# loli/medpy

Measured on AMD Instinct MI355X. Metric: Mvoxels/s graph-cut (build+solve), 512^3 6-conn; fraction of HBM roofline, higher is better.
Workload: dtype f64

## Files before the change

medpy_amd/csrc/mgc_common.h:

```cpp
#ifndef MGC_COMMON_H
#define MGC_COMMON_H

#include <stdint.h>

#if defined(__HIPCC__)
#define MGC_HD __host__ __device__ __forceinline__
#else
#define MGC_HD inline
#endif

#define MGC_T 8
#define MGC_TV 512
#define MGC_TF 64
#define MGC_HINF 0x3f3f3f3f

#define MGC_NDIR 6
#define MGC_MASK_SINK 0x40
#define MGC_NCOUNT 32
#define MGC_ST_SETTLED 1u
#define MGC_ST_SINK 2u
#define MGC_ST_DIRTY 4u
#define MGC_ST_SUSPECT 8u
#define MGC_ST_EXCESS 16u
#define MGC_ST_ALLINF 32u
#define MGC_ST_SOURCE 64u
#define MGC_WALL_WEIGHT 9.313225746154785e-10
#define MGC_WALL_VOXELS 24
#define MGC_ST_DEP_SHIFT 8
#define MGC_CNT_SINK_TILES 13
#define MGC_CNT_WALL_TILES 12
#define MGC_CNT_RADIAL_C 14
#define MGC_CNT_SOURCE_OPEN 15
#define MGC26_CNT_RADIAL_C 26
#define MGC26_CNT_SOURCE_OPEN 27
#define MGC_CNT_CHANGED 21
#define MGC_CNT_FILTER 22
#define MGC_CNT_FILTER_ACT 23
#define MGC_CNT_FILTER_B 30
#define MGC_CNT_FILTER_ACT_B 31
#define MGC_CNT_DEFERRED 28
#define MGC_CNT_WAVE_TILES 29
#define MGC_CNT_NOT_FULL 28

#if defined(__HIP_DEVICE_COMPILE__)
#define MGC_STORE_STREAM(p, v) __builtin_nontemporal_store((v), (p))
#else
#define MGC_STORE_STREAM(p, v) (*(p) = (v))
#endif

struct MgcLattice {
    int64_t dz, dy, dx;
    int64_t nvox;
    int gz, gy, gx;
    int ntiles;
    int tz_own_lo, tz_own_hi;
    int tz_global0;
    double*   rcap;
    double*   cap0;
    double*   excess;
    double*   sink;
    int32_t*  height;
    uint8_t*  rmask;
    uint32_t* rmask32;
    int       ndir;
    double*   obox;
    uint32_t* oflags;
    int32_t*  list[20];
    int32_t*  count;
    int32_t*  scount;
    int       nshard;
    int       shard_cap;
    uint32_t* stamp;
    uint32_t* rstamp;
    uint32_t* status;
    int       halo_max_rec;
    int32_t*  hshadow[2];
    unsigned long long* prof;
    const uint8_t* tsrc;
};

#ifndef MGC_NSHARD
#define MGC_NSHARD 1
#endif

MGC_HD int mgc_cnt_radial_c(const MgcLattice& L) { return L.ndir == 26 ? MGC26_CNT_RADIAL_C : MGC_CNT_RADIAL_C; }
MGC_HD int mgc_cnt_source_open(const MgcLattice& L) { return L.ndir == 26 ? MGC26_CNT_SOURCE_OPEN : MGC_CNT_SOURCE_OPEN; }

MGC_HD int32_t* mgc_counter(const MgcLattice& L, int c, int shard) { return L.scount + c * L.nshard + shard; }
// ... 112 lines not shown
```

medpy_amd/csrc/mgc_kernels.hip:

```cpp
#include <hip/hip_runtime.h>
#include <rccl/rccl.h>

#include <dlfcn.h>

#include <math.h>
#include <stdarg.h>
#include <stdio.h>
#include <stdlib.h>
#include <string.h>

#include <algorithm>
#include <chrono>
#include <map>
#include <string>
#include <mutex>
#include <thread>
#include <vector>

#include "../../include/medpy_hip.h"
#include "mgc_tile_ops.inl"
#include "mgc_tile_ops26.inl"
#include "mgc_wave_ops.inl"
#include "mgc_wave_ops26.inl"
#include "mgc_dt_ops.inl"
// ... 620 lines not shown
        __syncthreads();
    }
    x.flush_marks(L);
}

__global__ __launch_bounds__(MGC_TV) void k_absorb(MgcLattice L)
{
    __shared__ MgcTileShared S;
    GpuBlock x(S);
    for (int tile = blockIdx.x; tile < L.ntiles; tile += gridDim.x) {
        x.new_tile();
        mgc_absorb_tile(x, L, tile);
        __syncthreads();
    }
}

__global__ __launch_bounds__(MGC_TV) void k_relabel_all(MgcLattice L, uint32_t epoch, int next_list)
{
    __shared__ MgcTileShared S;
    GpuBlock x(S);
    int visited = 0;
    for (int tile = blockIdx.x; tile < L.ntiles; tile += gridDim.x) {
        x.new_tile();
        visited += (L.status[tile] >> 1) & 1u;
        mgc_relabel_tile(x, L, tile, epoch, next_list, true);
        __syncthreads();
    }
    if (threadIdx.x == 0 && visited) atomicAdd(&L.count[9], visited);
}

__global__ __launch_bounds__(MGC_TV) void k_relabel_list(MgcLattice L, int lst, uint32_t epoch, int next_list, int zero_list)
{
    __shared__ MgcTileShared S;
    GpuBlock x(S);
    MgcListView view;
    const int n = mgc_list_view(L, lst, view);
    if (blockIdx.x == 0 && threadIdx.x == 0 && n) atomicAdd(&L.count[9], n);
    mgc_clear_counter(L, zero_list);
    for (int i = blockIdx.x; i < n; i += gridDim.x) {
        x.new_tile();
        mgc_relabel_tile(x, L, mgc_list_at(L, lst, view, i), epoch, next_list, false);
        __syncthreads();
    }
}

__global__ void k_zero_counts(MgcLattice L, uint32_t mask)
{
    const int c = (int)threadIdx.x / MGC_NSHARD, sh = (int)threadIdx.x % MGC_NSHARD;
    if (!((mask >> c) & 1u)) return;
    if (sh == 0) L.count[c] = 0;
    if (sh < L.nshard) *mgc_counter(L, c, sh) = 0;
}

__global__ void k_status_or(MgcLattice L, uint32_t bits, uint32_t clear)
{
    const int tile = blockIdx.x * blockDim.x + threadIdx.x;
    if (tile < L.ntiles) L.status[tile] = (L.status[tile] & ~clear) | bits;
}

template <bool FULL>
__global__ __launch_bounds__(MGC_TV) void k_suspect_pass(MgcLattice L)
{
    const int bxn = (L.gx + 7) / 8, byn = (L.gy + 7) / 8, bzn = (L.gz + 7) / 8;
    const int t = threadIdx.x;
    bool any = false;
    for (int b = blockIdx.x; b < bxn * byn * bzn; b += gridDim.x) {
        const int bx = b % bxn, by = (b / bxn) % byn, bz = b / (bxn * byn);
        const int tz = bz * 8 + (t >> 6), ty = by * 8 + ((t >> 3) & 7), tx = bx * 8 + (t & 7);
        const bool in = tz < L.gz && ty < L.gy && tx < L.gx;
        const int tile = in ? mgc_tile_id(L, tz, ty, tx) : 0;
        for (int it = 0; it < 24; ++it) {
            const bool ch = in && (FULL ? mgc26_suspect_tile(L, tile) : mgc_suspect_tile(L, tile));
            any |= ch;
            __threadfence_block();
            if (!__syncthreads_or(ch)) break;
        }
    }
    if (any) L.count[MGC_CNT_CHANGED] = 1;
}

template <bool FULL>
__global__ __launch_bounds__(MGC_TV) void k_reset_suspect(MgcLattice L, uint32_t epoch, int list, int bricks)
{
    __shared__ MgcTileShared S;
    __shared__ int sel[MGC_TV];
    __shared__ int nsel;
    GpuBlock x(S);
    for (int base = blockIdx.x * MGC_TV; base < L.ntiles; base += gridDim.x * MGC_TV) {
        if (threadIdx.x == 0) nsel = 0;
        __syncthreads();
        const int mine = base + (int)threadIdx.x;
        if (mine < L.ntiles && (L.status[mine] & MGC_ST_SUSPECT)) sel[atomicAdd(&nsel, 1)] = mine;
        __syncthreads();
        const int n = nsel;
        for (int i = 0; i < n; ++i) {
            L.height[(int64_t)sel[i] * MGC_TV + threadIdx.x] = MGC_HINF;
            if (threadIdx.x < MGC_TF) mgc_shadow_reset(L, sel[i], (int)threadIdx.x);
        }
        if ((int)threadIdx.x < n) {
            const int tile = sel[threadIdx.x];
            L.status[tile] = (L.status[tile] & ~(MGC_ST_SUSPECT | MGC_ST_DIRTY | MGC_ST_SETTLED | (FULL ? MGC26_ST_DEP_MASK : (63u << MGC_ST_DEP_SHIFT)))) | MGC_ST_ALLINF;
            if (bricks) mgc_enqueue_brick(x, L, list, epoch, mgc_brick_of_tile(L, tile));
            else mgc_enqueue(x, L, list, L.rstamp, epoch, tile);
        }
        __syncthreads();
    }
}

__global__ void k_filter(MgcLattice L, int mode, int list, int cnt)
{
    for (int base = blockIdx.x * blockDim.x; base < L.ntiles; base += gridDim.x * blockDim.x) {
        const int tile = base + (int)threadIdx.x;
        bool take = false;
        if (tile < L.ntiles && mgc_owned(L, tile)) {
            if (mode == 0) {
                int tz, ty, tx;
                mgc_tile_coords(L, tile, tz, ty, tx);
                for (int f = 0; f < 6 && !take; ++f) {
                    const int nt = mgc_tile_nbr(L, tz, ty, tx, f);
                    take = nt >= 0 && ((L.oflags[nt] >> (f ^ 1)) & 1u);
                }
            } else if (mode == 1) {
                take = (L.status[tile] & (MGC_ST_EXCESS | MGC_ST_ALLINF)) == MGC_ST_EXCESS;
            } else if (mode == 3) {
                take = (L.status[tile] & MGC_ST_SINK) != 0;
            } else {
                take = (L.status[tile] & MGC_ST_SUSPECT) != 0;
            }
        }
        const unsigned long long m = __ballot(take);
        if (m) {
            int pos = 0;
            const int sh = (int)(blockIdx.x & (unsigned)(L.nshard - 1));
            if ((threadIdx.x & 63) == 0) pos = atomicAdd(mgc_counter(L, cnt, sh), __popcll(m));
            pos = __shfl(pos, 0);
            if (take) L.list[list][(int64_t)sh * L.shard_cap + pos + __popcll(m & ((1ull << (threadIdx.x & 63)) - 1ull))] = tile;
        }
    }
}

__global__ __launch_bounds__(MGC_TV) void k_relabel_first_list(MgcLattice L, int list, int cnt, uint32_t epoch, int next_list)
{
    __shared__ MgcTileShared S;
    GpuBlock x(S);
    MgcListView view;
    const int n = mgc_list_view(L, cnt, view);
    if (blockIdx.x == 0 && threadIdx.x == 0 && n) atomicAdd(&L.count[9], n);
    for (int i = blockIdx.x; i < n; i += gridDim.x) {
        x.new_tile();
        mgc_relabel_tile(x, L, mgc_list_at(L, list, view, i), epoch, next_list, true);
        __syncthreads();
    }
}

__global__ __launch_bounds__(256) void k_absorb_w(MgcLattice L, int list, int cnt, int clear_cnt)
{
    __shared__ MgcWaveShared S;
    GpuWave w(S);
// ... 1528 lines not shown
            *(void**)(&pop) = dlsym(dl, "roctxRangePop");
            if (push && pop) return;
            push = nullptr; pop = nullptr;
        }
    }
};
static MgcRoctx g_roctx;
static inline void mgc_range_push(const char* name)
{
    if (!g_roctx.tried) g_roctx.resolve();
    if (g_roctx.push) (void)g_roctx.push(name);
}
static inline void mgc_range_pop()
{
    if (g_roctx.pop) (void)g_roctx.pop();
}
struct MgcRange {
    explicit MgcRange(const char* name) { mgc_range_push(name); }
    ~MgcRange() { mgc_range_pop(); }
};
static std::string g_create_error;

struct mgc_graph {
    int device = 0;
    int ndim = 0;
    int64_t shape[3] = {1, 1, 1};
    int64_t nvox = 0;
    hipStream_t stream = nullptr;
    hipEvent_t ev[4] = {nullptr, nullptr, nullptr, nullptr};
    std::vector<hipEvent_t> ev_pool;
    struct OpSpan { int a, b, kind; };
    std::vector<hipEvent_t> op_ev;
    std::vector<OpSpan> op_spans;
    MgcLattice L{};
    void* d_image = nullptr; int img_dtype = 0; int term = MGC_TERM_NONE; double sigma = 0; double spacing[3] = {1, 1, 1};
    int has_spacing = 0;
    void* d_prob = nullptr; int prob_dtype = 0; double alpha = 0;
    void* d_lut = nullptr; int lut_n = 0;
    uint8_t* d_fg = nullptr; uint8_t* d_bg = nullptr;
    double* d_tr_in = nullptr; double flow_const_in = 0;
    MgcBuildArgs build_args{};
    int64_t n_edges = 0, n_runs = 0; int64_t* d_eslot = nullptr; double* d_eval = nullptr; int64_t* d_erun = nullptr;
    bool range_set = false; double range[3] = {0, 0, 0};
    bool edges_applied = false;
    double* d_dense = nullptr;
    std::vector<double*> dense_extra[26];
    int dense_given[26] = {};
    const double** d_dense_planes = nullptr;
    std::map<const void*, size_t> buf_cap;
    uint8_t* d_tsum = nullptr;
    uint8_t* d_tflags = nullptr;
    double* d_tr0 = nullptr; double* d_part = nullptr; double* d_part2 = nullptr; double* d_scalar = nullptr; uint8_t* d_labels = nullptr;
    int32_t* h_count = nullptr;
    double* h_scalar = nullptr;
    uint8_t* h_labels = nullptr; bool labels_on_host = false;
    uint8_t* d_labels_prev = nullptr; bool has_prev = false;
    bool built = false, solved = false;
    bool unconverged = false;
    bool labels_valid = false;
    void* d_vout = nullptr;
    uint16_t* d_dt16 = nullptr;
    uint16_t* d_ds16 = nullptr;
    int32_t* d_hexact = nullptr;
    bool radial_on = false;
    int radial_cycle_no = 0;
    bool all_residual = false;
    int exact_sink_tiles = 1;
    int sink_tiles = 0;
    int wall_tiles = 0;
    int radial_min_walls = 16;
    int sink_sweeps = 8;
    int use_bricks = 0;
    bool brick_mode = false;
    int use_dt = 1;
    int rank = 0, nranks = 1;
    int64_t plane0 = 0, plane1 = 0, own0 = 0, own1 = 0;
    int64_t gd0 = 0;
    uint16_t* d_carry[2] = {nullptr, nullptr};
    uint16_t* d_carry_in[2] = {nullptr, nullptr};
    uint16_t* dt_cur = nullptr;
    void* d_halo = nullptr; int64_t halo_cap = 0;
    ncclComm_t comm = nullptr; void* d_xchg[4] = {nullptr, nullptr, nullptr, nullptr}; int64_t xchg_cap = 0;
    int64_t* d_cnt64 = nullptr;
    double flow_const = 0.0, flow = 0.0;
    MgcSolveParams params = mgc_default_params();
    int grid_cap = 4096;
    int grid26_dis = 16384;
    int wave_kernels = 9;
    int wave_grid_dis = 0, wave_grid_rel = 0;
    int tk_dis = MGC_CNT_TICKET_DIS, tk_rel = MGC_CNT_TICKET_REL;
    int est_phase_tiles = 1 << 30;
    int sweeps_sparse26 = 5;
    int wave_grid26 = 0;
    bool rounds_set = false, sparse26_set = false, wave_set = false;
    bool w26_auto = false;
    int prepush = 1;
    int w26_passes = 2, w26_raises = 1, w26_flags = 0;
    int activate_exact_max = 4096;
    int wave_stagger = 0;
    int64_t launches[MGC_NLAUNCH] = {};
    int repeat_steps = 1;
    int repeat_min_tiles = 0;
    int repeat_flood_min_tiles = 200000;
    bool repeat_now = false;
    int wave_min_tiles = 512;
    uint32_t zero_mask = 0;
// ... 103 lines not shown
    }
    return hipFree(p);
}

template <class T>
static int mgc_alloc(mgc_handle h, T** p, int64_t count)
{
    MGC_HIP(h, mgc_dmalloc((void**)p, (size_t)count * sizeof(T)));
    h->device_bytes += count * (int64_t)sizeof(T);
    return MGC_OK;
}

static void mgc_fold_counts(mgc_handle h)
{
    const int ns = h->L.nshard;
    for (int c = 0; c < MGC_NCOUNT; ++c)
        for (int sh = 0; sh < ns; ++sh) h->h_count[c] += h->h_count[MGC_NCOUNT + c * ns + sh];
}

template <bool FULL>
struct HipDevT {
    mgc_handle h;
    hipError_t first_error = hipSuccess;
    float discharge_ms = 0.f, relabel_ms = 0.f, once_ms = 0.f;
    int64_t discharge_launches = 0, relabel_launches = 0, readbacks = 0;
    int last_discharged = -1;
    int suspect_batch() const { return 4; }
    bool labels_inexact() const { return false; }
    void range_push(const char* name) { mgc_range_push(name); }
    void range_pop() { mgc_range_pop(); }
    struct Span { int a, b, kind; };
    std::vector<Span> spans;
    void check(hipError_t e) { if (e != hipSuccess && first_error == hipSuccess) first_error = e; }
    int grid(int64_t n) const { return (int)(n < 1 ? 1 : (n < h->grid_cap ? n : h->grid_cap)); }
    void fill_heights_inf()
    {
        flush_zero();
        h->labels_valid = true;
        check(hipMemsetAsync(h->L.height, 0x3f, (size_t)h->L.ntiles * MGC_TV * sizeof(int32_t), h->stream));
        hipLaunchKernelGGL(k_status_or, dim3((h->L.ntiles + 255) / 256), dim3(256), 0, h->stream, h->L, (uint32_t)MGC_ST_ALLINF, (uint32_t)MGC_ST_SETTLED);
        for (int sd = 0; sd < 2; ++sd)
            if (h->L.hshadow[sd]) check(hipMemsetAsync(h->L.hshadow[sd], 0x3f, (size_t)h->L.gy * h->L.gx * MGC_TF * sizeof(int32_t), h->stream));
    }
    void flush_zero()
    {
        if (h->pending_zero >= 0) h->zero_mask |= 1u << h->pending_zero;
        h->pending_zero = -1;
        if (h->zero_mask) {
            hipLaunchKernelGGL(k_zero_counts, dim3(1), dim3(MGC_NCOUNT * MGC_NSHARD), 0, h->stream, h->L, h->zero_mask);
            check(hipGetLastError());
        }
        h->zero_mask = 0;
    }
    void zero_count(int i)
    {
        if (i == last_discharged) { flush_zero(); h->pending_zero = i; last_discharged = -1; return; }
        if (h->pending_zero >= 0) { h->zero_mask |= 1u << h->pending_zero; h->pending_zero = -1; }
        h->zero_mask |= 1u << i;
    }
    void read_counts(int* out)
    {
        flush_zero();
        check(hipMemcpyAsync(h->h_count, h->L.count, MGC_NCOUNT * (1 + MGC_NSHARD) * sizeof(int32_t), hipMemcpyDeviceToHost, h->stream));
        check(hipStreamSynchronize(h->stream));
        mgc_fold_counts(h);
        memcpy(out, h->h_count, MGC_NCOUNT * sizeof(int32_t));
        readbacks++;
        if (!FULL) {
            int m = out[6] / 2;
            for (int i = 0; i < 4; ++i) m = out[i] > m ? out[i] : m;
            h->est_phase_tiles = m;
        } else {
            int m = out[MGC26_CNT_ACTIVE] / 8;
            for (int i = 0; i < MGC26_NLIST; ++i) m = out[i] > m ? out[i] : m;
            h->est_phase_tiles = m;
        }
    }
    int filter_grid() const { const int g = (h->L.ntiles + 255) / 256; return g < 1024 ? g : 1024; }
    int fslot(int which) const { return which == 0 ? (h->filt[0] ? MGC_CNT_FILTER_B : MGC_CNT_FILTER) : (h->filt[1] ? MGC_CNT_FILTER_ACT_B : MGC_CNT_FILTER_ACT); }
    int fnext(int which) const { return which == 0 ? (h->filt[0] ? MGC_CNT_FILTER : MGC_CNT_FILTER_B) : (h->filt[1] ? MGC_CNT_FILTER_ACT : MGC_CNT_FILTER_ACT_B); }
    void filter_done(int which, bool consumer_cleared_next)
    {
        if (!consumer_cleared_next) zero_count(fnext(which));
        h->filt[which] ^= 1;
    }
    void absorb_all()
    {
        flush_zero();
        if constexpr (FULL) return;
        else if (!(h->use_filters & 1)) { hipLaunchKernelGGL(k_absorb, dim3(grid(h->L.ntiles)), dim3(MGC_TV), 0, h->stream, h->L); check(hipGetLastError()); }
        else {
            flush_zero();
            hipLaunchKernelGGL(k_filter, dim3(filter_grid()), dim3(256), 0, h->stream, h->L, 0, 6, fslot(0));
            if (h->wave_kernels & 1) hipLaunchKernelGGL(k_absorb_w, dim3(grid((h->L.ntiles + 3) / 4)), dim3(256), 0, h->stream, h->L, 6, fslot(0), fnext(0));
            else hipLaunchKernelGGL(k_absorb_list, dim3(grid(h->L.ntiles)), dim3(MGC_TV), 0, h->stream, h->L, 6, fslot(0), fnext(0));
            filter_done(0, true);
            check(hipGetLastError());
        }
    }
    void relabel_all(uint32_t epoch, int next)
    {
        flush_zero();
        h->brick_mode = false;
        const int id = time_begin(1);
        if constexpr (FULL) hipLaunchKernelGGL(k26_relabel_all, dim3(grid(h->L.ntiles)), dim3(MGC_TV), 0, h->stream, h->L, epoch, next);
        else if (!(h->use_filters & 1)) { hipLaunchKernelGGL(k_relabel_all, dim3(grid(h->L.ntiles)), dim3(MGC_TV), 0, h->stream, h->L, epoch, next); h->launches[MGC_LAUNCH_RELABEL_TILE]++; }
        else {
            flush_zero();
            hipLaunchKernelGGL(k_filter, dim3(filter_grid()), dim3(256), 0, h->stream, h->L, 3, 6, fslot(0));
            if (h->wave_kernels & 8) { hipLaunchKernelGGL(k_relabel_v, dim3(grid(h->L.ntiles)), dim3(MGC_TV / MGC_RELABEL_V), 0, h->stream, h->L, 6, fslot(0), epoch, next, fnext(0), 1); filter_done(0, true); h->launches[MGC_LAUNCH_RELABEL_V]++; }
            else if (h->wave_kernels & 2) { hipLaunchKernelGGL(k_relabel_w, dim3(h->wave_grid_rel), dim3(MGCW_LANES), 0, h->stream, h->L, 6, fslot(0), epoch, next, -1, 1, h->tk_rel); h->tk_rel ^= 1; filter_done(0, false); h->launches[MGC_LAUNCH_RELABEL_W]++; }
            else { hipLaunchKernelGGL(k_relabel_first_list, dim3(grid(h->L.ntiles)), dim3(MGC_TV), 0, h->stream, h->L, 6, fslot(0), epoch, next); filter_done(0, false); h->launches[MGC_LAUNCH_RELABEL_TILE]++; }
        }
        check(hipGetLastError());
        time_end(id);
        relabel_launches++;
    }
    template <int AXIS, int SEED, int FINAL>
    void dt_axis(const void* in, uint16_t* T, int c_min)
// ... 61 lines not shown
        check(hipMemsetAsync(L.count + mgc_cnt_radial_c(L), 0x3f, sizeof(int32_t), h->stream));
        hipLaunchKernelGGL(k_dt_cmin, g(L.ntiles), blk, 0, h->stream, L);
        dt_axis<0, 2, 0>((const void*)L.excess, T, 0);
        dt_axis<1, 0, 0>((const void*)T, T, 0);
        dt_axis<2, 0, 2>((const void*)T, T, c_min);
        std::swap(h->L.height, h->d_hexact);
        check(hipGetLastError());
        time_end(id);
        relabel_launches++;
        return true;
    }
    void radial_save_exact()
    {
        flush_zero();
        check(hipMemcpyAsync(h->d_hexact, h->L.height, (size_t)h->L.ntiles * MGC_TV * sizeof(int32_t), hipMemcpyDeviceToDevice, h->stream));
    }
    void radial_restore_exact()
    {
        flush_zero();
        std::swap(h->L.height, h->d_hexact);
    }
    void radial_lower(int c_min)
    {
        flush_zero();
        const int id = time_begin(2);
        hipLaunchKernelGGL(k_dt_lower, dim3(grid((h->L.ntiles + 3) / 4)), dim3(256), 0, h->stream, h->L, (const uint16_t*)h->d_ds16, c_min);
        check(hipGetLastError());
        time_end(id);
        relabel_launches++;
    }
    void source_open()
    {
        flush_zero();
        hipLaunchKernelGGL(k_source_open, dim3(grid((h->L.ntiles + 3) / 4)), dim3(256), 0, h->stream, h->L);
        check(hipGetLastError());
    }
    void relabel_list(int lst, uint32_t epoch, int next, int zero_list = -1)
    {
        flush_zero();
        const int id = time_begin(1);
        if (!FULL && h->brick_mode) { hipLaunchKernelGGL(k_relabel_b, dim3(grid(mgc_brick_count(h->L))), dim3(MGC_TV), 0, h->stream, h->L, lst, epoch, next, zero_list); h->launches[MGC_LAUNCH_RELABEL_TILE]++; }
        else if constexpr (FULL) hipLaunchKernelGGL(k26_relabel_list, dim3(grid(h->L.ntiles)), dim3(MGC_TV), 0, h->stream, h->L, lst, epoch, next);
        else if (h->wave_kernels & 8) { hipLaunchKernelGGL(k_relabel_v, dim3(grid(h->L.ntiles)), dim3(MGC_TV / MGC_RELABEL_V), 0, h->stream, h->L, lst, lst, epoch, next, zero_list, 0); h->launches[MGC_LAUNCH_RELABEL_V]++; }
        else if (h->wave_kernels & 2) { hipLaunchKernelGGL(k_relabel_w, dim3(h->wave_grid_rel), dim3(MGCW_LANES), 0, h->stream, h->L, lst, lst, epoch, next, zero_list, 0, h->tk_rel); h->tk_rel ^= 1; h->launches[MGC_LAUNCH_RELABEL_W]++; }
        else { hipLaunchKernelGGL(k_relabel_list, dim3(grid(h->L.ntiles)), dim3(MGC_TV), 0, h->stream, h->L, lst, epoch, next, zero_list); h->launches[MGC_LAUNCH_RELABEL_TILE]++; }
        check(hipGetLastError());
        time_end(id);
        relabel_launches++;
    }
    void suspect_pass()
    {
        flush_zero();
        const int nb = ((h->L.gx + 7) / 8) * ((h->L.gy + 7) / 8) * ((h->L.gz + 7) / 8);
        hipLaunchKernelGGL(k_suspect_pass<FULL>, dim3(nb < 4096 ? nb : 4096), dim3(MGC_TV), 0, h->stream, h->L);
        check(hipGetLastError());
    }
    void reset_suspect(uint32_t epoch, int list)
    {
        flush_zero();
        const int id = time_begin(1);
        h->brick_mode = !FULL && h->use_bricks && h->nranks == 1 && !(h->use_filters & 4);
        if (FULL || !(h->use_filters & 4)) hipLaunchKernelGGL(k_reset_suspect<FULL>, dim3(grid((h->L.ntiles + MGC_TV - 1) / MGC_TV)), dim3(MGC_TV), 0, h->stream, h->L, epoch, list, h->brick_mode ? 1 : 0);
        else {
            flush_zero();
            hipLaunchKernelGGL(k_filter, dim3(filter_grid()), dim3(256), 0, h->stream, h->L, 2, 6, fslot(0));
            hipLaunchKernelGGL(k_reset_suspect_list, dim3(grid(h->L.ntiles)), dim3(MGC_TV), 0, h->stream, h->L, 6, fslot(0), epoch, list);
            filter_done(0, false);
        }
        check(hipGetLastError());
        time_end(id);
        relabel_launches++;
    }
    void activate_all(uint32_t phase)
    {
        flush_zero();
        if constexpr (FULL) {
            if (h->L.nshard == 1 && (h->use_filters & 2)) hipLaunchKernelGGL(k26_activate_w, dim3(grid((h->L.ntiles + 3) / 4)), dim3(256), 0, h->stream, h->L, phase);
            else hipLaunchKernelGGL(k26_activate, dim3(grid(h->L.ntiles)), dim3(MGC_TV), 0, h->stream, h->L, phase);
        }
        else if (!(h->use_filters & 2)) hipLaunchKernelGGL(k_activate, dim3(grid(h->L.ntiles)), dim3(MGC_TV), 0, h->stream, h->L, phase);
        else {
            flush_zero();
            hipLaunchKernelGGL(k_filter, dim3(filter_grid()), dim3(256), 0, h->stream, h->L, 1, 7, fslot(1));
            if (h->wave_kernels & 1) { hipLaunchKernelGGL(k_activate_w, dim3(grid((h->L.ntiles + 3) / 4)), dim3(256), 0, h->stream, h->L, 7, fslot(1), phase, h->activate_exact_max, fnext(1)); filter_done(1, true); }
            else { hipLaunchKernelGGL(k_activate_list, dim3(grid(h->L.ntiles)), dim3(MGC_TV), 0, h->stream, h->L, 7, fslot(1), phase); filter_done(1, false); }
        }
        check(hipGetLastError());
    }
    void discharge(int lst, uint32_t phase, int cycles, int sweeps)
    {
        const int zero_idx = h->pending_zero;
        h->pending_zero = -1;
        flush_zero();
        const bool wave_form = !FULL && (h->wave_kernels & 1) && h->est_phase_tiles >= h->wave_min_tiles;
        const int id = time_begin(FULL || wave_form ? 0 : 3);
        if constexpr (FULL) {
            if (h->sweeps_sparse26 > 0 && (int64_t)h->est_phase_tiles * 40 < h->L.ntiles) sweeps = h->sweeps_sparse26;
            if (((h->wave_kernels & 32) || h->w26_auto) && cycles < 0) {
                hipLaunchKernelGGL(k26_discharge_w, dim3(h->wave_grid26), dim3(MGCW_LANES), 0, h->stream, h->L, lst, phase, sweeps, h->w26_auto ? 1 : h->w26_passes, h->w26_raises, h->w26_flags, h->tk_dis, zero_idx);
                h->tk_dis ^= 1;
                h->launches[MGC_LAUNCH_DISCHARGE26_W]++;
            }
            else if (h->wave_kernels & 16) { hipLaunchKernelGGL(k26_discharge_v, dim3(grid(h->L.ntiles)), dim3(MGC_TV / 2), 0, h->stream, h->L, lst, phase, cycles, sweeps, zero_idx); h->launches[MGC_LAUNCH_DISCHARGE26_V]++; }
            else { hipLaunchKernelGGL(k26_discharge, dim3(h->grid26_dis > 0 ? (h->grid26_dis < h->L.ntiles ? h->grid26_dis : h->L.ntiles) : grid(h->L.ntiles)), dim3(MGC_TV), 0, h->stream, h->L, lst, phase, cycles, sweeps, zero_idx); h->launches[MGC_LAUNCH_DISCHARGE26]++; }
        }
        else if (wave_form) {
            const bool exact_sink = h->exact_sink_tiles == 2 || (h->exact_sink_tiles == 1 && 2 * (int64_t)h->sink_tiles > h->L.ntiles);
// ... 396 lines not shown
        L.tz_own_lo = slab->own_lo; L.tz_own_hi = slab->own_hi; L.tz_global0 = slab->tz_global0;
        h->rank = slab->rank; h->nranks = slab->nranks;
        h->plane0 = slab->plane0; h->plane1 = slab->plane1; h->own0 = slab->own0; h->own1 = slab->own1;
    } else {
        h->plane0 = h->own0 = 0; h->plane1 = h->own1 = L.dz;
    }
    h->gd0 = gd0 > 0 ? gd0 : L.dz;
    *out = h;
    MGC_HIP(h, hipSetDevice(device));
    MGC_HIP(h, hipStreamCreateWithFlags(&h->stream, hipStreamNonBlocking));
    for (int i = 0; i < 4; ++i) MGC_HIP(h, hipEventCreate(&h->ev[i]));
    const int64_t nt = L.ntiles, nv = nt * MGC_TV;
    int rc;
    if ((rc = mgc_alloc(h, &L.rcap, nv * L.ndir))) return rc;
    L.cap0 = nullptr;
    if ((rc = mgc_alloc(h, &L.excess, nv))) return rc;
    if ((rc = mgc_alloc(h, &L.sink, nv))) return rc;
    if ((rc = mgc_alloc(h, &L.height, nv))) return rc;
    if (L.ndir == 6) {
        if ((rc = mgc_alloc(h, &L.rmask, nv))) return rc;
        if ((rc = mgc_alloc(h, &L.obox, nt * 6 * MGC_TF))) return rc;
    } else {
        if ((rc = mgc_alloc(h, &L.rmask32, nv))) return rc;
    }
    if ((rc = mgc_alloc(h, &L.oflags, nt))) return rc;
    if (slab && L.ndir == 6) {
        for (int sd = 0; sd < 2; ++sd) {
            if ((rc = mgc_alloc(h, &L.hshadow[sd], (int64_t)L.gy * L.gx * MGC_TF))) return rc;
            MGC_HIP(h, hipMemsetAsync(L.hshadow[sd], 0x3f, (size_t)L.gy * L.gx * MGC_TF * sizeof(int32_t), h->stream));
        }
    }
    L.nshard = 1;
    {
        const int64_t T = gy * gx;
        L.halo_max_rec = (int)(T / 8 > 64 ? T / 8 : (T < 64 ? T : 64));
    }
    L.shard_cap = (int)nt;
    for (int i = 0; i < (L.ndir == 6 ? 8 : 18); ++i)
        if ((rc = mgc_alloc(h, &L.list[i], nt * MGC_NSHARD))) return rc;
    if ((rc = mgc_alloc(h, &L.count, (int64_t)MGC_NCOUNT * (1 + MGC_NSHARD)))) return rc;
    L.scount = L.count + MGC_NCOUNT;
    if ((rc = mgc_alloc(h, &L.stamp, nt))) return rc;
    if ((rc = mgc_alloc(h, &L.rstamp, nt))) return rc;
    if ((rc = mgc_alloc(h, &L.status, nt))) return rc;
    if ((rc = mgc_alloc(h, &h->d_tr0, nv))) return rc;
    if ((rc = mgc_alloc(h, &h->d_tflags, nt))) return rc;
    if ((rc = mgc_alloc(h, &h->d_tsum, nt))) return rc;
    if ((rc = mgc_alloc(h, &h->d_part, nt > 4096 ? nt : (int64_t)4096))) return rc;
    if ((rc = mgc_alloc(h, &h->d_part2, (int64_t)256))) return rc;
    if ((rc = mgc_alloc(h, &h->d_scalar, (int64_t)8))) return rc;
    if ((rc = mgc_alloc(h, &h->d_labels, n))) return rc;
    MGC_HIP(h, hipHostMalloc((void**)&h->h_count, MGC_NCOUNT * (1 + MGC_NSHARD) * sizeof(int32_t), hipHostMallocDefault));
    MGC_HIP(h, hipHostMalloc((void**)&h->h_scalar, 8 * sizeof(double), hipHostMallocDefault));
    MGC_HIP(h, hipMemsetAsync(L.count, 0, MGC_NCOUNT * (1 + MGC_NSHARD) * sizeof(int32_t), h->stream));
    MGC_HIP(h, hipStreamSynchronize(h->stream));
    if (const char* wv = getenv("MEDPY_HIP_WAVE")) { h->wave_kernels = atoi(wv); h->wave_set = true; }
    {
        hipDeviceProp_t prop;
        MGC_HIP(h, hipGetDeviceProperties(&prop, device));
        int per_cu_dis = 0, per_cu_rel = 0;
        MGC_HIP(h, hipOccupancyMaxActiveBlocksPerMultiprocessor(&per_cu_dis, k_discharge_w<1>, MGCW_LANES, 0));
        MGC_HIP(h, hipOccupancyMaxActiveBlocksPerMultiprocessor(&per_cu_rel, k_relabel_w, MGCW_LANES, 0));
        h->wave_grid_dis = prop.multiProcessorCount * (per_cu_dis > 0 ? per_cu_dis : 8);
        h->wave_grid_rel = prop.multiProcessorCount * (per_cu_rel > 0 ? per_cu_rel : 16);
        int per_cu_26 = 0;
        MGC_HIP(h, hipOccupancyMaxActiveBlocksPerMultiprocessor(&per_cu_26, k26_discharge_w, MGCW_LANES, 0));
        h->wave_grid26 = prop.multiProcessorCount * (per_cu_26 > 0 ? per_cu_26 : 4);
    }
    return MGC_OK;
}

int mgc_create(int ndim, const int64_t* shape, int connectivity, int device, mgc_handle* out)
{
    return mgc_create_impl(ndim, shape, connectivity, device, nullptr, out);
}

int mgc_create_slab(int ndim, const int64_t* gshape, int connectivity, int device, int rank, int nranks, mgc_handle* out)
{
    if (!out) return mgc_fail(nullptr, MGC_ERR_INVALID, "mgc_create_slab: out is NULL");
    *out = nullptr;
    if (ndim != 3 || !gshape) return mgc_fail(nullptr, MGC_ERR_UNSUPPORTED, "mgc_create_slab: slabs need a 3-D volume");
    if (nranks < 1 || rank < 0 || rank >= nranks) return mgc_fail(nullptr, MGC_ERR_INVALID, "bad rank %d of %d", rank, nranks);
    MgcSlabSpec sp;
    if (mgc_slab_spec(gshape[0], rank, nranks, &sp)) return mgc_fail(nullptr, MGC_ERR_INVALID, "cannot cut %lld planes into %d slabs", (long long)gshape[0], nranks);
    const int64_t lshape[3] = {sp.plane1 - sp.plane0, gshape[1], gshape[2]};
    return mgc_create_impl(3, lshape, connectivity, device, &sp, out, gshape[0]);
}

int mgc_slab_info(mgc_handle h, int64_t* info)
{
    if (!h || !info) return MGC_ERR_INVALID;
    info[0] = h->plane0; info[1] = h->plane1; info[2] = h->own0; info[3] = h->own1;
    info[4] = h->L.tz_own_lo > 0; info[5] = h->L.tz_own_hi < h->L.gz; info[6] = (int64_t)h->L.gy * h->L.gx; info[7] = h->nranks;
    return MGC_OK;
}

int mgc_solver_op(mgc_handle h, int op, int64_t a0, int64_t a1, int64_t a2, int64_t a3)
{
    if (!h) return MGC_ERR_INVALID;
    if (!h->built) return mgc_fail(h, MGC_ERR_STATE, "mgc_solver_op before mgc_build");
    MGC_HIP(h, hipSetDevice(h->device));
    if (h->L.ndir == MGC26_NDIR) return mgc_solver_op_on<HipDevT<true>>(h, op, a0, a1, a2, a3);
    return mgc_solver_op_on<HipDevT<false>>(h, op, a0, a1, a2, a3);
}

int mgc_read_counts(mgc_handle h, int32_t* out)
// ... 335 lines not shown
}

extern "C" {

int mgc_solve_slabs(mgc_handle* hs, int n, const mgc_transport* t, mgc_slab_stats* out)
{
    if (!hs || n < 1 || !hs[0]) return MGC_ERR_INVALID;
    mgc_handle h0 = hs[0];
    for (int i = 0; i < n; ++i) {
        if (!hs[i]) return MGC_ERR_INVALID;
        if (!hs[i]->built) return mgc_fail(h0, MGC_ERR_STATE, "mgc_solve_slabs before mgc_build (slab %d)", i);
        if (hs[i]->device != h0->device || hs[i]->L.ndir != h0->L.ndir || hs[i]->nranks != h0->nranks || hs[i]->gd0 != h0->gd0 || hs[i]->L.dy != h0->L.dy || hs[i]->L.dx != h0->L.dx)
            return mgc_fail(h0, MGC_ERR_INVALID, "mgc_solve_slabs: the local slabs are cut from one volume and live on one device");
        if (n > 1 && hs[i]->rank != i) return mgc_fail(h0, MGC_ERR_INVALID, "mgc_solve_slabs: all slabs of the volume, in rank order");
    }
    if (n > 1 && n != h0->nranks) return mgc_fail(h0, MGC_ERR_INVALID, "mgc_solve_slabs: %d local slabs of a volume cut into %d (either all of them or this rank's one)", n, h0->nranks);
    if (n == 1 && h0->nranks > 1) {
        if (!h0->comm && !(t && t->exchange && t->allreduce && t->send && t->recv))
            return mgc_fail(h0, MGC_ERR_STATE, "mgc_solve_slabs: this slab has neighbours in other processes: call mgc_comm_init first (RCCL), or pass the four callbacks of a host transport");
    }
    MGC_HIP(h0, hipSetDevice(h0->device));
    MgcRange range_("mgc_solve_slabs");
    float ms = 0.f;
    MGC_HIP(h0, hipEventRecord(h0->ev[0], h0->stream));
    const int rc = h0->L.ndir == MGC26_NDIR ? mgc_solve_slabs_on<HipDev26>(hs, n, t, mgc_layout26(), out) : mgc_solve_slabs_on<HipDev>(hs, n, t, mgc_layout6(), out);
    if (rc == MGC_OK) {
        MGC_HIP(h0, hipEventRecord(h0->ev[1], h0->stream));
        MGC_HIP(h0, hipStreamSynchronize(h0->stream));
        MGC_HIP(h0, hipEventElapsedTime(&ms, h0->ev[0], h0->ev[1]));
        for (int i = 0; i < n; ++i) hs[i]->stats.solve_ms = ms;
    }
    return rc;
}

int mgc_solve_slab(mgc_handle h, mgc_slab_stats* out) { return mgc_solve_slabs(&h, 1, nullptr, out); }

int mgc_destroy(mgc_handle h)
{
    if (!h) return MGC_OK;
    (void)hipSetDevice(h->device);
    if (h->stream) (void)hipStreamSynchronize(h->stream);
    if (h->comm && g_rccl.CommDestroy) (void)g_rccl.CommDestroy(h->comm);
    MgcLattice& L = h->L;
    void* ptrs[] = {L.rcap, L.cap0, L.excess, L.sink, L.height, L.rmask, L.rmask32, L.obox, L.oflags, L.list[0], L.list[1], L.list[2],
                    L.list[3], L.list[4], L.list[5], L.list[6], L.list[7], L.list[8], L.list[9], L.list[10], L.list[11], L.list[12],
                    L.list[13], L.list[14], L.list[15], L.list[16], L.list[17], L.count, L.stamp, L.rstamp, L.status, h->d_tr0, h->d_part, h->d_part2, h->d_scalar,
                    h->d_labels, h->d_labels_prev, h->d_tflags, h->d_tsum, h->d_image, h->d_lut, h->d_prob, h->d_fg, h->d_bg, h->d_tr_in, h->d_eslot, h->d_eval, h->d_erun, h->d_dense, (void*)h->d_dense_planes, L.hshadow[0], L.hshadow[1], h->d_vout, h->d_dt16, h->d_ds16, h->d_hexact, h->d_halo, h->d_xchg[0], h->d_xchg[1], h->d_xchg[2], h->d_xchg[3], h->d_cnt64, h->d_carry[0], h->d_carry[1], h->d_carry_in[0], h->d_carry_in[1]};
    for (void* p : ptrs)
        if (p) (void)mgc_dfree(p);
    for (auto& planes : h->dense_extra)
        for (double* p : planes) (void)mgc_dfree(p);
    if (h->h_count) (void)hipHostFree(h->h_count);
    if (h->h_scalar) (void)hipHostFree(h->h_scalar);
    free(h->h_labels);
    for (int i = 0; i < 4; ++i)
        if (h->ev[i]) (void)hipEventDestroy(h->ev[i]);
    for (hipEvent_t e : h->ev_pool) (void)hipEventDestroy(e);
    for (hipEvent_t e : h->op_ev) (void)hipEventDestroy(e);
    if (h->stream) (void)hipStreamDestroy(h->stream);
    delete h;
    return MGC_OK;
}

#ifndef MGC_STAGE_THREADS
#define MGC_STAGE_THREADS 4
#define MGC_STAGE_THREADS_UP 4
#endif
#define MGC_STAGE_CHUNK ((size_t)8 << 20)
struct MgcStage {
    std::mutex lock;
    void* pinned = nullptr;
    hipStream_t stream[8] = {nullptr, nullptr, nullptr, nullptr, nullptr, nullptr, nullptr, nullptr};
    bool failed = false;
};
static MgcStage g_stage[16];

static hipError_t mgc_staged_copy(mgc_handle h, void* dev, void* host, size_t bytes, bool to_device)
{
    if (bytes < 4 * MGC_STAGE_CHUNK) {
        hipError_t e = to_device ? hipMemcpyAsync(dev, host, bytes, hipMemcpyHostToDevice, h->stream) : hipMemcpyAsync(host, dev, bytes, hipMemcpyDeviceToHost, h->stream);
        return e != hipSuccess ? e : hipStreamSynchronize(h->stream);
    }
    static const int env_threads = getenv("MEDPY_HIP_STAGE_THREADS") ? atoi(getenv("MEDPY_HIP_STAGE_THREADS")) : -1;
    const int want = env_threads >= 0 ? env_threads : (to_device ? MGC_STAGE_THREADS_UP : MGC_STAGE_THREADS);
    if (want == 0) {
        hipError_t e = to_device ? hipMemcpyAsync(dev, host, bytes, hipMemcpyHostToDevice, h->stream) : hipMemcpyAsync(host, dev, bytes, hipMemcpyDeviceToHost, h->stream);
        return e != hipSuccess ? e : hipStreamSynchronize(h->stream);
    }
    const int NT = want > 8 ? 8 : want, SLOTS = 2;
    MgcStage& G = g_stage[h->device & 15];
    std::lock_guard<std::mutex> guard(G.lock);
    if (!G.pinned && !G.failed) {
        if (hipHostMalloc(&G.pinned, (size_t)8 * SLOTS * MGC_STAGE_CHUNK, hipHostMallocDefault) != hipSuccess) {
            (void)hipGetLastError();
            G.pinned = nullptr;
            G.failed = true;
        } else {
            for (int i = 0; i < 8; ++i) if (hipStreamCreateWithFlags(&G.stream[i], hipStreamNonBlocking) != hipSuccess) G.stream[i] = nullptr;
        }
    }
    if (!G.pinned) {
        hipError_t e = to_device ? hipMemcpyAsync(dev, host, bytes, hipMemcpyHostToDevice, h->stream) : hipMemcpyAsync(host, dev, bytes, hipMemcpyDeviceToHost, h->stream);
        return e != hipSuccess ? e : hipStreamSynchronize(h->stream);
    }
    hipError_t first = hipStreamSynchronize(h->stream);
    if (first != hipSuccess) return first;
// ... 1068 lines not shown
```

Before: 7629.

## Poll mapped host memory for counter readback and track per-pass closure flags

```diff
diff --git a/medpy_amd/csrc/mgc_common.h b/medpy_amd/csrc/mgc_common.h
--- a/medpy_amd/csrc/mgc_common.h
+++ b/medpy_amd/csrc/mgc_common.h
@@ -34,6 +34,7 @@
 #define MGC26_CNT_RADIAL_C 26
 #define MGC26_CNT_SOURCE_OPEN 27
 #define MGC_CNT_CHANGED 21
+#define MGC_CNT_CHANGED_PASS 16
 #define MGC_CNT_FILTER 22
 #define MGC_CNT_FILTER_ACT 23
 #define MGC_CNT_FILTER_B 30
diff --git a/medpy_amd/csrc/mgc_kernels.hip b/medpy_amd/csrc/mgc_kernels.hip
--- a/medpy_amd/csrc/mgc_kernels.hip
+++ b/medpy_amd/csrc/mgc_kernels.hip
@@ -696,6 +696,14 @@
     if (sh < L.nshard) *mgc_counter(L, c, sh) = 0;
 }
 
+__global__ __launch_bounds__(64) void k_look(const int32_t* count, int32_t* out, int n, uint32_t seq)
+{
+    for (int i = (int)threadIdx.x; i < n; i += 64) out[i] = count[i];
+    __threadfence_system();
+    asm volatile("s_waitcnt vmcnt(0)" ::: "memory");
+    if (threadIdx.x == 0) __hip_atomic_store((uint32_t*)(out + n), seq, __ATOMIC_RELEASE, __HIP_MEMORY_SCOPE_SYSTEM);
+}
+
 __global__ void k_status_or(MgcLattice L, uint32_t bits, uint32_t clear)
 {
     const int tile = blockIdx.x * blockDim.x + threadIdx.x;
@@ -703,7 +711,7 @@
 }
 
 template <bool FULL>
-__global__ __launch_bounds__(MGC_TV) void k_suspect_pass(MgcLattice L)
+__global__ __launch_bounds__(MGC_TV) void k_suspect_pass(MgcLattice L, int changed)
 {
     const int bxn = (L.gx + 7) / 8, byn = (L.gy + 7) / 8, bzn = (L.gz + 7) / 8;
     const int t = threadIdx.x;
@@ -720,7 +728,7 @@
             if (!__syncthreads_or(ch)) break;
         }
     }
-    if (any) L.count[MGC_CNT_CHANGED] = 1;
+    if (any) L.count[changed] = 1;
 }
 
 template <bool FULL>
@@ -741,13 +749,18 @@
             L.height[(int64_t)sel[i] * MGC_TV + threadIdx.x] = MGC_HINF;
             if (threadIdx.x < MGC_TF) mgc_shadow_reset(L, sel[i], (int)threadIdx.x);
         }
+        bool left_out = false;
         if ((int)threadIdx.x < n) {
             const int tile = sel[threadIdx.x];
-            L.status[tile] = (L.status[tile] & ~(MGC_ST_SUSPECT | MGC_ST_DIRTY | MGC_ST_SETTLED | (FULL ? MGC26_ST_DEP_MASK : (63u << MGC_ST_DEP_SHIFT)))) | MGC_ST_ALLINF;
+            const uint32_t st = L.status[tile];
+            const bool seeds = FULL || bricks || mgc_reset_seeds_tile(L, tile, st);
+            L.status[tile] = (st & ~(MGC_ST_SUSPECT | MGC_ST_DIRTY | MGC_ST_SETTLED | (FULL ? MGC26_ST_DEP_MASK : (63u << MGC_ST_DEP_SHIFT)))) | MGC_ST_ALLINF;
             if (bricks) mgc_enqueue_brick(x, L, list, epoch, mgc_brick_of_tile(L, tile));
-            else mgc_enqueue(x, L, list, L.rstamp, epoch, tile);
-        }
-        __syncthreads();
+            else if (seeds) mgc_enqueue(x, L, list, L.rstamp, epoch, tile);
+            left_out = !seeds;
+        }
+        const int nleft = __syncthreads_count(left_out);
+        if (!FULL && threadIdx.x == 0 && nleft) atomicAdd(&L.count[9], nleft);
     }
 }
 
@@ -2382,6 +2395,9 @@
     uint8_t* d_tflags = nullptr;
     double* d_tr0 = nullptr; double* d_part = nullptr; double* d_part2 = nullptr; double* d_scalar = nullptr; uint8_t* d_labels = nullptr;
     int32_t* h_count = nullptr;
+    int32_t* h_look = nullptr;
+    int32_t* d_look = nullptr;
+    uint32_t look_seq = 0;
     double* h_scalar = nullptr;
     uint8_t* h_labels = nullptr; bool labels_on_host = false;
     uint8_t* d_labels_prev = nullptr; bool has_prev = false;
@@ -2591,8 +2607,15 @@
         }
         h->zero_mask = 0;
     }
+    int closure_pass = -1;
+    int closure_word = MGC_CNT_CHANGED;
+    bool closure_words() const { return !FULL && h->nranks == 1; }
     void zero_count(int i)
     {
+        if (i == MGC_CNT_CHANGED && closure_words()) {
+            closure_pass = 0;
+            h->zero_mask |= 15u << MGC_CNT_CHANGED_PASS;
+        }
         if (i == last_discharged) { flush_zero(); h->pending_zero = i; last_discharged = -1; return; }
         if (h->pending_zero >= 0) { h->zero_mask |= 1u << h->pending_zero; h->pending_zero = -1; }
         h->zero_mask |= 1u << i;
@@ -2600,10 +2623,30 @@
     void read_counts(int* out)
     {
         flush_zero();
-        check(hipMemcpyAsync(h->h_count, h->L.count, MGC_NCOUNT * (1 + MGC_NSHARD) * sizeof(int32_t), hipMemcpyDeviceToHost, h->stream));
-        check(hipStreamSynchronize(h->stream));
+        const int nw = MGC_NCOUNT * (1 + MGC_NSHARD);
+        if (h->d_look && h->nranks == 1) {
+            const uint32_t seq = ++h->look_seq;
+            hipLaunchKernelGGL(k_look, dim3(1), dim3(64), 0, h->stream, (const int32_t*)h->L.count, h->d_look, nw, seq);
+            check(hipGetLastError());
+            const uint32_t* word = (const uint32_t*)(h->h_look + nw);
+            bool seen = false;
+            const auto t0 = std::chrono::steady_clock::now();
+            for (uint32_t spin = 1; !(seen = __atomic_load_n(word, __ATOMIC_ACQUIRE) == seq); ++spin) {
+#if !defined(__HIP_DEVICE_COMPILE__) && (defined(__x86_64__) || defined(__i386__))
+                __builtin_ia32_pause();
+#endif
+                if ((spin & 255u) == 0 && std::chrono::steady_clock::now() - t0 > std::chrono::milliseconds(50)) break;
+            }
+            if (!seen) check(hipStreamSynchronize(h->stream));
+            memcpy(h->h_count, h->h_look, nw * sizeof(int32_t));
+        } else {
+            check(hipMemcpyAsync(h->h_count, h->L.count, nw * sizeof(int32_t), hipMemcpyDeviceToHost, h->stream));
+            check(hipStreamSynchronize(h->stream));
+        }
         mgc_fold_counts(h);
         memcpy(out, h->h_count, MGC_NCOUNT * sizeof(int32_t));
+        if (closure_pass > 0) out[MGC_CNT_CHANGED] = out[closure_word];
+        closure_pass = -1;
         readbacks++;
         if (!FULL) {
             int m = out[6] / 2;
@@ -2771,7 +2814,11 @@
     {
         flush_zero();
         const int nb = ((h->L.gx + 7) / 8) * ((h->L.gy + 7) / 8) * ((h->L.gz + 7) / 8);
-        hipLaunchKernelGGL(k_suspect_pass<FULL>, dim3(nb < 4096 ? nb : 4096), dim3(MGC_TV), 0, h->stream, h->L);
+        if (closure_pass >= 0) {
+            closure_word = MGC_CNT_CHANGED_PASS + (closure_pass < 3 ? closure_pass : 3);
+            closure_pass++;
+        }
+        hipLaunchKernelGGL(k_suspect_pass<FULL>, dim3(nb < 4096 ? nb : 4096), dim3(MGC_TV), 0, h->stream, h->L, closure_pass >= 0 ? closure_word : MGC_CNT_CHANGED);
         check(hipGetLastError());
     }
     void reset_suspect(uint32_t epoch, int list)
@@ -3274,6 +3321,9 @@
     if ((rc = mgc_alloc(h, &h->d_labels, n))) return rc;
     MGC_HIP(h, hipHostMalloc((void**)&h->h_count, MGC_NCOUNT * (1 + MGC_NSHARD) * sizeof(int32_t), hipHostMallocDefault));
     MGC_HIP(h, hipHostMalloc((void**)&h->h_scalar, 8 * sizeof(double), hipHostMallocDefault));
+    MGC_HIP(h, hipHostMalloc((void**)&h->h_look, (MGC_NCOUNT * (1 + MGC_NSHARD) + 1) * sizeof(int32_t), hipHostMallocMapped | hipHostMallocCoherent));
+    memset(h->h_look, 0, (MGC_NCOUNT * (1 + MGC_NSHARD) + 1) * sizeof(int32_t));
+    MGC_HIP(h, hipHostGetDevicePointer((void**)&h->d_look, h->h_look, 0));
     MGC_HIP(h, hipMemsetAsync(L.count, 0, MGC_NCOUNT * (1 + MGC_NSHARD) * sizeof(int32_t), h->stream));
     MGC_HIP(h, hipStreamSynchronize(h->stream));
     if (const char* wv = getenv("MEDPY_HIP_WAVE")) { h->wave_kernels = atoi(wv); h->wave_set = true; }
@@ -3715,6 +3765,7 @@
         for (double* p : planes) (void)mgc_dfree(p);
     if (h->h_count) (void)hipHostFree(h->h_count);
     if (h->h_scalar) (void)hipHostFree(h->h_scalar);
+    if (h->h_look) (void)hipHostFree(h->h_look);
     free(h->h_labels);
     for (int i = 0; i < 4; ++i)
         if (h->ev[i]) (void)hipEventDestroy(h->ev[i]);
```

Result: faster. 7825, median of 6 (+2.6%).
